# nv-tlabs/GEN3C

Hardware: NVIDIA H100
Metric: denoise-steps/sec, 7B DiT, 121-frame 720p latent (higher is better)
Workload: dtype bf16

## Files before the change

gen3c_b200/csrc/common.cuh:

```cuda
#pragma once
#include <cuda.h>
#include <cuda_bf16.h>
#include <cuda_runtime.h>
#include <stdint.h>
#include <stdio.h>

#include "../../include/gen3c_b200.h"
#include "wgmma_ops.cuh"

namespace g3c {

void set_error(const char* fmt, ...);
int cuda_fail(cudaError_t e, const char* what, const char* file, int line);
#define G3C_CUDA(x)                                                         \
  do {                                                                      \
    cudaError_t _e = (x);                                                   \
    if (_e != cudaSuccess) return ::g3c::cuda_fail(_e, #x, __FILE__, __LINE__); \
  } while (0)
#define G3C_REQUIRE(cond, ...)        \
  do {                                \
    if (!(cond)) {                    \
      ::g3c::set_error(__VA_ARGS__);  \
      return G3C_EINVAL;       \
    }                                 \
  } while (0)

int make_tmap_bf16_sw128(CUtensorMap* out, const void* base, int rank, const uint64_t* dims,
                         const uint64_t* strides_bytes, const uint32_t* box,
                         CUtensorMapDataType dtype = CU_TENSOR_MAP_DATA_TYPE_BFLOAT16);
int make_tmap_f32_sw128(CUtensorMap* out, const void* base, const uint64_t* dims,
                        const uint64_t* strides_bytes, const uint32_t* box);

int sm_count();

#ifdef __CUDACC__
__device__ __forceinline__ uint32_t smem_u32(const void* p) {
  return static_cast<uint32_t>(__cvta_generic_to_shared(p));
}
__device__ __forceinline__ uint32_t lane_id() { return threadIdx.x & 31; }
__device__ __forceinline__ uint32_t warp_id() { return __shfl_sync(0xffffffffu, threadIdx.x >> 5, 0); }

__device__ __forceinline__ bool elect_one() {
  uint32_t pred = 0;
  asm volatile(
      "{\n\t.reg .pred P;\n\t"
      "elect.sync _|P, 0xffffffff;\n\t"
      "selp.b32 %0, 1, 0, P;\n\t}\n"
      : "=r"(pred));
  return pred != 0;
}

__device__ __forceinline__ void mbar_init(uint64_t* bar, uint32_t count) {
  asm volatile("mbarrier.init.shared::cta.b64 [%0], %1;\n" ::"r"(smem_u32(bar)), "r"(count));
}
__device__ __forceinline__ void fence_barrier_init() {
  asm volatile("fence.mbarrier_init.release.cluster;\n" ::: "memory");
}
__device__ __forceinline__ void fence_proxy_async() {
  asm volatile("fence.proxy.async.shared::cta;\n" ::: "memory");
}
__device__ __forceinline__ void mbar_expect_tx(uint64_t* bar, uint32_t bytes) {
  asm volatile("mbarrier.arrive.expect_tx.shared::cta.b64 _, [%0], %1;\n" ::"r"(smem_u32(bar)),
               "r"(bytes)
               : "memory");
}
__device__ __forceinline__ void mbar_arrive(uint64_t* bar) {
  asm volatile("mbarrier.arrive.shared::cta.b64 _, [%0];\n" ::"r"(smem_u32(bar)) : "memory");
}
#ifndef G3C_MBAR_SUSPEND_NS
#define G3C_MBAR_SUSPEND_NS 0
#endif
__device__ __forceinline__ bool mbar_try_wait(uint64_t* bar, uint32_t parity) {
  uint32_t ok;
#if G3C_MBAR_SUSPEND_NS > 0
  asm volatile(
      "{\n\t.reg .pred P;\n\t"
      "mbarrier.try_wait.parity.shared::cta.b64 P, [%1], %2, %3;\n\t"
      "selp.b32 %0, 1, 0, P;\n\t}\n"
      : "=r"(ok)
      : "r"(smem_u32(bar)), "r"(parity), "r"((uint32_t)G3C_MBAR_SUSPEND_NS)
      : "memory");
#else
  asm volatile(
      "{\n\t.reg .pred P;\n\t"
      "mbarrier.try_wait.parity.shared::cta.b64 P, [%1], %2;\n\t"
      "selp.b32 %0, 1, 0, P;\n\t}\n"
      : "=r"(ok)
      : "r"(smem_u32(bar)), "r"(parity)
      : "memory");
#endif
  return ok != 0;
}
__device__ __forceinline__ bool mbar_test(uint64_t* bar, uint32_t parity) {
  uint32_t ok;
  asm volatile(
      "{\n\t.reg .pred P;\n\t"
      "mbarrier.test_wait.parity.shared::cta.b64 P, [%1], %2;\n\t"
      "selp.b32 %0, 1, 0, P;\n\t}\n"
      : "=r"(ok)
      : "r"(smem_u32(bar)), "r"(parity)
      : "memory");
  return ok != 0;
}
#ifndef G3C_MBAR_TIMEOUT_NS
#define G3C_MBAR_TIMEOUT_NS 4000000000ull
#endif
__device__ __forceinline__ uint64_t global_timer_ns() {
  uint64_t t;
  asm volatile("mov.u64 %0, %%globaltimer;\n" : "=l"(t));
  return t;
}
#ifdef G3C_MBAR_DEBUG
#define G3C_MBAR_TIMEOUT_ACTION(bar, parity)                                                                 \
  do {                                                                                                       \
    printf("g3c: mbarrier timeout block(%d,%d) thread %d bar@%u parity %u\n", blockIdx.x, blockIdx.y,        \
           threadIdx.x, bar, parity);                                                                        \
    __trap();                                                                                                \
  } while (0)
#else
#define G3C_MBAR_TIMEOUT_ACTION(bar, parity) asm volatile("trap;\n")
#endif
__device__ __forceinline__ void mbar_wait(uint64_t* bar, uint32_t parity) {
  if (mbar_try_wait(bar, parity)) return;
  uint32_t spins = 0;
  uint64_t t0 = 0;
  while (!mbar_try_wait(bar, parity)) {
    if ((++spins & 0xFFFu) == 0) {
      uint64_t now = global_timer_ns();
      if (t0 == 0) t0 = now;
      else if (now - t0 > G3C_MBAR_TIMEOUT_NS) G3C_MBAR_TIMEOUT_ACTION(smem_u32(bar), parity);
    }
  }
}

__device__ __forceinline__ void mbar_wait_ns(uint64_t* bar, uint32_t parity, unsigned long long timeout_ns) {
  if (mbar_try_wait(bar, parity)) return;
  uint32_t spins = 0;
  uint64_t t0 = 0;
  while (!mbar_try_wait(bar, parity)) {
    if ((++spins & 0xFFFu) == 0) {
      uint64_t now = global_timer_ns();
      if (t0 == 0) t0 = now;
      else if (now - t0 > timeout_ns) G3C_MBAR_TIMEOUT_ACTION(smem_u32(bar), parity);
    }
  }
}

__device__ __forceinline__ void mbar_wait_ns_or_exit(uint64_t* bar, uint32_t parity, unsigned long long timeout_ns) {
  if (mbar_try_wait(bar, parity)) return;
  uint32_t spins = 0;
  uint64_t t0 = 0;
  while (!mbar_try_wait(bar, parity)) {
    if ((++spins & 0xFFFu) == 0) {
      uint64_t now = global_timer_ns();
      if (t0 == 0) t0 = now;
      else if (now - t0 > timeout_ns) asm volatile("exit;\n");
    }
  }
}

__device__ __forceinline__ void tma_prefetch_desc(const CUtensorMap* m) {
  asm volatile("prefetch.tensormap [%0];\n" ::"l"(reinterpret_cast<uint64_t>(m)) : "memory");
}
__device__ __forceinline__ void tma_load_2d(void* smem_dst, const CUtensorMap* m, uint64_t* bar,
                                            int c0, int c1) {
  asm volatile(
      "cp.async.bulk.tensor.2d.shared::cluster.global.mbarrier::complete_tx::bytes"
      " [%0], [%1, {%3, %4}], [%2];\n" ::"r"(smem_u32(smem_dst)),
      "l"(reinterpret_cast<uint64_t>(m)), "r"(smem_u32(bar)), "r"(c0), "r"(c1)
      : "memory");
}
__device__ __forceinline__ void tma_load_3d(void* smem_dst, const CUtensorMap* m, uint64_t* bar,
                                            int c0, int c1, int c2) {
  asm volatile(
      "cp.async.bulk.tensor.3d.shared::cluster.global.mbarrier::complete_tx::bytes"
      " [%0], [%1, {%3, %4, %5}], [%2];\n" ::"r"(smem_u32(smem_dst)),
      "l"(reinterpret_cast<uint64_t>(m)), "r"(smem_u32(bar)), "r"(c0), "r"(c1), "r"(c2)
      : "memory");
}

__device__ __forceinline__ void tma_store_2d(const CUtensorMap* m, const void* smem_src, int c0, int c1) {
  asm volatile("cp.async.bulk.tensor.2d.global.shared::cta.bulk_group [%0, {%2, %3}], [%1];\n" ::"l"(
                   reinterpret_cast<uint64_t>(m)),
               "r"(smem_u32(smem_src)), "r"(c0), "r"(c1)
               : "memory");
}
__device__ __forceinline__ void tma_reduce_add_2d(const CUtensorMap* m, const void* smem_src, int c0, int c1) {
  asm volatile("cp.reduce.async.bulk.tensor.2d.global.shared::cta.add.bulk_group [%0, {%2, %3}], [%1];\n" ::"l"(
                   reinterpret_cast<uint64_t>(m)),
               "r"(smem_u32(smem_src)), "r"(c0), "r"(c1)
               : "memory");
}
__device__ __forceinline__ void tma_store_commit() { asm volatile("cp.async.bulk.commit_group;\n" ::: "memory"); }
template <int N>
__device__ __forceinline__ void tma_store_wait_read() {
  asm volatile("cp.async.bulk.wait_group.read %0;\n" ::"n"(N) : "memory");
}
template <int N>
__device__ __forceinline__ void tma_store_wait_all() {
  asm volatile("cp.async.bulk.wait_group %0;\n" ::"n"(N) : "memory");
}

__device__ __forceinline__ void wgmma_fence() { asm volatile("wgmma.fence.sync.aligned;\n" ::: "memory"); }
__device__ __forceinline__ void wgmma_commit() { asm volatile("wgmma.commit_group.sync.aligned;\n" ::: "memory"); }
template <int N>
__device__ __forceinline__ void wgmma_wait() {
  asm volatile("wgmma.wait_group.sync.aligned %0;\n" ::"n"(N) : "memory");
}
template <int N>
__device__ __forceinline__ void fence_regs(float (&r)[N]) {
#pragma unroll
  for (int i = 0; i < N; ++i) asm volatile("" : "+f"(r[i])::"memory");
}
template <int N>
__device__ __forceinline__ void fence_regs(uint32_t (&r)[N]) {
#pragma unroll
  for (int i = 0; i < N; ++i) asm volatile("" : "+r"(r[i])::"memory");
}

__device__ __forceinline__ uint64_t make_sdesc_sw128(uint32_t smem_addr) {
  uint64_t d = 0;
  d |= static_cast<uint64_t>((smem_addr & 0x3FFFFu) >> 4);
  d |= static_cast<uint64_t>(1) << 16;
  d |= static_cast<uint64_t>(1024u >> 4) << 32;
  d |= static_cast<uint64_t>(1) << 62;
  return d;
}
__device__ __forceinline__ uint64_t make_sdesc_sw128_mn(uint32_t smem_addr, uint32_t mn_block_bytes) {
  uint64_t d = 0;
  d |= static_cast<uint64_t>((smem_addr & 0x3FFFFu) >> 4);
  d |= static_cast<uint64_t>((mn_block_bytes >> 4) & 0x3FFFu) << 16;
  d |= static_cast<uint64_t>(1024u >> 4) << 32;
  d |= static_cast<uint64_t>(1) << 62;
  return d;
}
__device__ __forceinline__ uint64_t sdesc_advance(uint64_t d, uint32_t bytes) {
  return d + static_cast<uint64_t>(bytes >> 4);
}

template <int N>
__device__ __forceinline__ void setmaxnreg_dec() {
  asm volatile("setmaxnreg.dec.sync.aligned.u32 %0;\n" ::"n"(N));
}
template <int N>
__device__ __forceinline__ void setmaxnreg_inc() {
  asm volatile("setmaxnreg.inc.sync.aligned.u32 %0;\n" ::"n"(N));
}

__device__ __forceinline__ uint32_t pack_bf16x2(float lo, float hi) {
  __nv_bfloat162 v = __floats2bfloat162_rn(lo, hi);
  return *reinterpret_cast<uint32_t*>(&v);
}
__device__ __forceinline__ float warp_max(float v) {
#pragma unroll
  for (int o = 16; o > 0; o >>= 1) v = fmaxf(v, __shfl_xor_sync(0xffffffffu, v, o));
  return v;
}
__device__ __forceinline__ float warp_sum(float v) {
#pragma unroll
  for (int o = 16; o > 0; o >>= 1) v += __shfl_xor_sync(0xffffffffu, v, o);
  return v;
}
#endif

}
```

gen3c_b200/csrc/gemm_wgmma.cu:

```cuda
#include <cstdlib>
#include <cstring>

#include "kernels.h"

namespace g3c {

constexpr int BM = 128;
constexpr int BK = 64;
constexpr int WG_K = 16;
template <bool kFp8>
constexpr int kBlockK = kFp8 ? 2 * BK : BK;
constexpr int GEMM_THREADS = 384;

struct GemmParams {
  int M, N, K;
  int ldd;
  void* D;
  const float* gate;
  int num_m_blk, num_n_blk, num_k_blk;
  int super_n;
  const float* nr_gamma;
  const float* nr_cs;
  float nr_eps;
  const float* scale_a;
  const float* scale_b;
};

constexpr int EPI_NORM_ROPE_BF16 = 4;

template <int BN>
struct GemmSmem {
  static constexpr int kABytes = BM * BK * 2;
  static constexpr int kBBytes = BN * BK * 2;
  static constexpr int kStageBytes = kABytes + kBBytes;
  static constexpr int kStages = (192 * 1024) / kStageBytes;
  static constexpr int kBarBytes = 256;
  static constexpr int kTotal = kStages * kStageBytes + kBarBytes + 1024;
};

__device__ __forceinline__ float gelu_erf(float x) {
  return 0.5f * x * (1.0f + erff(x * 0.70710678118654752440f));
}

__device__ __forceinline__ void tile_coords(const GemmParams& p, int tile, int& m_blk, int& n_blk) {
  int per_super = p.num_m_blk * p.super_n;
  int sc = tile / per_super;
  int rem = tile - sc * per_super;
  int n0 = sc * p.super_n;
  int width = p.num_n_blk - n0 < p.super_n ? p.num_n_blk - n0 : p.super_n;
  m_blk = rem / width;
  n_blk = n0 + rem - m_blk * width;
}

template <int BN>
__device__ __forceinline__ void epilogue_norm_rope(const float (&acc)[BN / 2], const GemmParams& p, int row_a, int col_q,
                                                   int n_base) {
#pragma unroll
  for (int hd = 0; hd < BN / 128; ++hd) {
    if (n_base + hd * 128 >= p.N) break;
    float ss[2] = {0.f, 0.f};
#pragma unroll
    for (int i = 16 * hd; i < 16 * hd + 16; ++i) {
      ss[0] = fmaf(acc[4 * i], acc[4 * i], fmaf(acc[4 * i + 1], acc[4 * i + 1], ss[0]));
      ss[1] = fmaf(acc[4 * i + 2], acc[4 * i + 2], fmaf(acc[4 * i + 3], acc[4 * i + 3], ss[1]));
    }
#pragma unroll
    for (int h = 0; h < 2; ++h) {
      ss[h] += __shfl_xor_sync(0xffffffffu, ss[h], 1);
      ss[h] += __shfl_xor_sync(0xffffffffu, ss[h], 2);
    }
#pragma unroll
    for (int h = 0; h < 2; ++h) {
      const int row = row_a + 8 * h;
      if (row >= p.M) continue;
      const float rstd = rsqrtf(ss[h] * (1.0f / 128.0f) + p.nr_eps);
      const float* cs = p.nr_cs ? p.nr_cs + (size_t)row * 128 : nullptr;
      __nv_bfloat16* dptr = reinterpret_cast<__nv_bfloat16*>(p.D) + (size_t)row * p.ldd + n_base + hd * 128;
#pragma unroll
      for (int i = 0; i < 8; ++i) {
        const int c = 8 * i + col_q;
        const float2 ga = *reinterpret_cast<const float2*>(p.nr_gamma + c);
        const float2 gb = *reinterpret_cast<const float2*>(p.nr_gamma + 64 + c);
        const int ia = 4 * (16 * hd + i) + 2 * h, ib = 4 * (16 * hd + i + 8) + 2 * h;
        float a[2] = {acc[ia] * (rstd * ga.x), acc[ia + 1] * (rstd * ga.y)};
        float b[2] = {acc[ib] * (rstd * gb.x), acc[ib + 1] * (rstd * gb.y)};
        if (cs) {
          const float2 co = *reinterpret_cast<const float2*>(cs + c);
          const float2 si = *reinterpret_cast<const float2*>(cs + 64 + c);
          const float cv[2] = {co.x, co.y}, sv[2] = {si.x, si.y};
#pragma unroll
          for (int e = 0; e < 2; ++e) {
            const float n = a[e] * cv[e] - b[e] * sv[e], m = b[e] * cv[e] + a[e] * sv[e];
            a[e] = n;
            b[e] = m;
          }
        }
        *reinterpret_cast<uint32_t*>(dptr + c) = pack_bf16x2(a[0], a[1]);
        *reinterpret_cast<uint32_t*>(dptr + 64 + c) = pack_bf16x2(b[0], b[1]);
      }
    }
  }
}

template <int BN>
__device__ __forceinline__ void dequantise(float (&acc)[BN / 2], const GemmParams& p, int row_a, int col_q, int n_base) {
  float sa[2];
#pragma unroll
  for (int h = 0; h < 2; ++h) sa[h] = row_a + 8 * h < p.M ? p.scale_a[row_a + 8 * h] : 0.f;
#pragma unroll
  for (int i = 0; i < BN / 8; ++i) {
    const int col = n_base + 8 * i + col_q;
    float2 sb = make_float2(0.f, 0.f);
    if (col + 1 < p.N) sb = *reinterpret_cast<const float2*>(p.scale_b + col);
    else if (col < p.N) sb.x = p.scale_b[col];
#pragma unroll
    for (int h = 0; h < 2; ++h) {
      acc[4 * i + 2 * h] = acc[4 * i + 2 * h] * sa[h] * sb.x;
      acc[4 * i + 2 * h + 1] = acc[4 * i + 2 * h + 1] * sa[h] * sb.y;
    }
  }
}

template <int BN, int EPI>
__device__ __forceinline__ void epilogue(const float (&acc)[BN / 2], const GemmParams& p, int row_a, int col_q,
                                         int n_base) {
  if constexpr (EPI == EPI_NORM_ROPE_BF16) {
    epilogue_norm_rope<BN>(acc, p, row_a, col_q, n_base);
  } else {
#pragma unroll
    for (int h = 0; h < 2; ++h) {
      const int row = row_a + 8 * h;
      if (row >= p.M) continue;
#pragma unroll
      for (int i = 0; i < BN / 8; ++i) {
        const int col = n_base + 8 * i + col_q;
        if (col >= p.N) continue;
        const bool pair = col + 1 < p.N;
        float v0 = acc[4 * i + 2 * h], v1 = acc[4 * i + 2 * h + 1];
        if constexpr (EPI == G3C_EPI_BF16 || EPI == G3C_EPI_GELU_BF16) {
          if constexpr (EPI == G3C_EPI_GELU_BF16) {
            v0 = gelu_erf(v0);
            v1 = gelu_erf(v1);
          }
          __nv_bfloat16* dptr = reinterpret_cast<__nv_bfloat16*>(p.D) + (size_t)row * p.ldd + col;
          if (pair) *reinterpret_cast<uint32_t*>(dptr) = pack_bf16x2(v0, v1);
          else dptr[0] = __float2bfloat16_rn(v0);
        } else {
          float* dptr = reinterpret_cast<float*>(p.D) + (size_t)row * p.ldd + col;
          if constexpr (EPI == G3C_EPI_GATED_RESIDUAL_F32) {
            if (pair) {
              const float2 g = *reinterpret_cast<const float2*>(p.gate + col);
              float2 x = *reinterpret_cast<float2*>(dptr);
              x.x = fmaf(g.x, v0, x.x);
              x.y = fmaf(g.y, v1, x.y);
              *reinterpret_cast<float2*>(dptr) = x;
            } else {
              dptr[0] = fmaf(p.gate[col], v0, dptr[0]);
            }
          } else {
            if (pair) *reinterpret_cast<float2*>(dptr) = make_float2(v0, v1);
            else dptr[0] = v0;
          }
        }
      }
    }
  }
}

template <int BN, int EPI, bool kFp8>
__global__ void __launch_bounds__(GEMM_THREADS, 1)
    k_gemm(const __grid_constant__ CUtensorMap tmA, const __grid_constant__ CUtensorMap tmB, const GemmParams p) {
  using S = GemmSmem<BN>;
  constexpr int kStages = S::kStages;
  extern __shared__ uint8_t smem_raw[];
  uint8_t* smem = reinterpret_cast<uint8_t*>((reinterpret_cast<uintptr_t>(smem_raw) + 1023) &
                                             ~static_cast<uintptr_t>(1023));
  uint8_t* smem_a = smem;
  uint8_t* smem_b = smem + kStages * S::kABytes;
  uint64_t* bars = reinterpret_cast<uint64_t*>(smem + kStages * S::kStageBytes);
  uint64_t* full = bars;
  uint64_t* empty = bars + kStages;

  const uint32_t wg = threadIdx.x / 128;
  const uint32_t tid = threadIdx.x % 128;

  if (threadIdx.x == 0) {
    tma_prefetch_desc(&tmA);
    tma_prefetch_desc(&tmB);
    for (int i = 0; i < kStages; ++i) {
      mbar_init(&full[i], 1);
      mbar_init(&empty[i], 2);
    }
    fence_barrier_init();
  }
  __syncthreads();

  const int num_tiles = p.num_m_blk * p.num_n_blk;

  if (wg == 0) {
    setmaxnreg_dec<40>();
    if (tid == 0) {
      uint32_t stage = 0, phase = 0;
      for (int tile = blockIdx.x; tile < num_tiles; tile += gridDim.x) {
        int m_blk, n_blk;
        tile_coords(p, tile, m_blk, n_blk);
        for (int kb = 0; kb < p.num_k_blk; ++kb) {
          mbar_wait(&empty[stage], phase ^ 1);
          mbar_expect_tx(&full[stage], S::kStageBytes);
          tma_load_2d(smem_a + stage * S::kABytes, &tmA, &full[stage], kb * kBlockK<kFp8>, m_blk * BM);
          tma_load_2d(smem_b + stage * S::kBBytes, &tmB, &full[stage], kb * kBlockK<kFp8>, n_blk * BN);
          if (++stage == kStages) {
            stage = 0;
            phase ^= 1;
          }
        }
      }
    }
  } else {
    setmaxnreg_inc<232>();
    const uint32_t c = wg - 1;
    const uint32_t warp = tid / 32, lane = tid % 32;
    uint32_t stage = 0, phase = 0;
    float acc[BN / 2];
    for (int tile = blockIdx.x; tile < num_tiles; tile += gridDim.x) {
      int m_blk, n_blk;
      tile_coords(p, tile, m_blk, n_blk);
      if constexpr (kFp8) {
        static_assert(BN <= 128, "fp8 tiles hold two accumulator sets");
        float part[BN / 2];
#pragma unroll
        for (int i = 0; i < BN / 2; ++i) acc[i] = 0.f;
        for (int kb = 0; kb < p.num_k_blk; ++kb) {
          mbar_wait(&full[stage], phase);
          const uint64_t da = make_sdesc_sw128(smem_u32(smem_a + stage * S::kABytes + c * 64 * 128));
          const uint64_t db = make_sdesc_sw128(smem_u32(smem_b + stage * S::kBBytes));
          wgmma_fence();
#pragma unroll
          for (int k = 0; k < BK / WG_K; ++k) {
            const uint64_t a = sdesc_advance(da, k * WG_K * 2), b = sdesc_advance(db, k * WG_K * 2);
            if constexpr (BN == 128) wgmma_ss_n128_e4m3(part, a, b, k != 0 ? 1u : 0u);
            else wgmma_ss_n64_e4m3(part, a, b, k != 0 ? 1u : 0u);
          }
          wgmma_commit();
          wgmma_wait<0>();
          fence_regs(part);
          if (tid == 0) mbar_arrive(&empty[stage]);
#pragma unroll
          for (int i = 0; i < BN / 2; ++i) acc[i] += part[i];
          if (++stage == kStages) {
            stage = 0;
            phase ^= 1;
          }
        }
      } else {
        uint32_t prev_stage = 0;
        for (int kb = 0; kb < p.num_k_blk; ++kb) {
          mbar_wait(&full[stage], phase);
          const uint64_t da = make_sdesc_sw128(smem_u32(smem_a + stage * S::kABytes + c * 64 * 128));
          const uint64_t db = make_sdesc_sw128(smem_u32(smem_b + stage * S::kBBytes));
          wgmma_fence();
#pragma unroll
          for (int k = 0; k < BK / WG_K; ++k) {
            const uint64_t a = sdesc_advance(da, k * WG_K * 2), b = sdesc_advance(db, k * WG_K * 2);
            const uint32_t accumulate = (kb | k) != 0 ? 1u : 0u;
            if constexpr (BN == 256) wgmma_ss_n256(acc, a, b, accumulate);
            else if constexpr (BN == 128) wgmma_ss_n128(acc, a, b, accumulate);
            else wgmma_ss_n64(acc, a, b, accumulate);
          }
          wgmma_commit();
          wgmma_wait<1>();
          fence_regs(acc);
          if (kb > 0 && tid == 0) mbar_arrive(&empty[prev_stage]);
          prev_stage = stage;
          if (++stage == kStages) {
            stage = 0;
            phase ^= 1;
          }
        }
        wgmma_wait<0>();
        fence_regs(acc);
        if (tid == 0) mbar_arrive(&empty[prev_stage]);
      }
      const int row_a = m_blk * BM + (int)(c * 64 + warp * 16 + lane / 4), col_q = (int)(2 * (lane % 4));
      if constexpr (kFp8) dequantise<BN>(acc, p, row_a, col_q, n_blk * BN);
      epilogue<BN, EPI>(acc, p, row_a, col_q, n_blk * BN);
    }
  }
}

template <int BN, int EPI, bool kFp8>
static int launch_gemm(const CUtensorMap& tmA, const CUtensorMap& tmB, const GemmParams& p, cudaStream_t st) {
  using S = GemmSmem<BN>;
  static bool configured = false;
  if (!configured) {
    G3C_CUDA(cudaFuncSetAttribute(k_gemm<BN, EPI, kFp8>, cudaFuncAttributeMaxDynamicSharedMemorySize, S::kTotal));
    configured = true;
  }
  int tiles = p.num_m_blk * p.num_n_blk;
  int grid = tiles < sm_count() ? tiles : sm_count();
  k_gemm<BN, EPI, kFp8><<<grid, GEMM_THREADS, S::kTotal, st>>>(tmA, tmB, p);
  G3C_CUDA(cudaGetLastError());
  return G3C_OK;
}

template <int BN, bool kFp8>
static int dispatch_epi(int epi, const CUtensorMap& tmA, const CUtensorMap& tmB, const GemmParams& p, cudaStream_t st) {
  switch (epi) {
    case G3C_EPI_BF16: return launch_gemm<BN, G3C_EPI_BF16, kFp8>(tmA, tmB, p, st);
    case G3C_EPI_GELU_BF16: return launch_gemm<BN, G3C_EPI_GELU_BF16, kFp8>(tmA, tmB, p, st);
    case G3C_EPI_GATED_RESIDUAL_F32: return launch_gemm<BN, G3C_EPI_GATED_RESIDUAL_F32, kFp8>(tmA, tmB, p, st);
    case G3C_EPI_F32: return launch_gemm<BN, G3C_EPI_F32, kFp8>(tmA, tmB, p, st);
    case EPI_NORM_ROPE_BF16:
      if constexpr (BN >= 128) return launch_gemm<BN, EPI_NORM_ROPE_BF16, kFp8>(tmA, tmB, p, st);
      break;
  }
  set_error("gemm: unknown epilogue %d", epi);
  return G3C_EINVAL;
}

static int gemm_any(const void* A, const void* B, const float* scale_a, const float* scale_b, void* D, int M, int N,
                    int K, int lda, int ldb, int ldd, int epilogue, const float* gate, int block_n, cudaStream_t st,
                    const NormRope* norm_rope) {
  const bool fp8 = scale_a != nullptr;
  G3C_REQUIRE(A && B && D, "gemm: null operand");
  G3C_REQUIRE(epilogue >= G3C_EPI_BF16 && epilogue <= G3C_EPI_F32, "gemm: unknown epilogue %d", epilogue);
  if (norm_rope) {
    G3C_REQUIRE(epilogue == G3C_EPI_BF16 && N % 128 == 0 && norm_rope->gamma,
                "gemm: the RMSNorm/RoPE epilogue needs the bf16 epilogue, N %% 128 == 0 and a gain vector");
    G3C_REQUIRE((reinterpret_cast<uintptr_t>(norm_rope->gamma) & 15) == 0 &&
                    (reinterpret_cast<uintptr_t>(norm_rope->cs) & 15) == 0,
                "gemm: RMSNorm gain / RoPE table must be 16-byte aligned");
    epilogue = EPI_NORM_ROPE_BF16;
  }
  G3C_REQUIRE(M > 0 && N > 0 && K > 0, "gemm: bad shape %dx%dx%d", M, N, K);
  if (fp8)
    G3C_REQUIRE(K % 16 == 0 && lda % 16 == 0 && ldb % 16 == 0, "gemm_fp8: K/lda/ldb must be multiples of 16");
  else
    G3C_REQUIRE(K % 8 == 0 && lda % 8 == 0 && ldb % 8 == 0, "gemm: K/lda/ldb must be multiples of 8");
  G3C_REQUIRE(lda >= K && ldb >= K && ldd >= N, "gemm: leading dimension smaller than extent");
  if (epilogue == G3C_EPI_BF16 || epilogue == G3C_EPI_GELU_BF16 || epilogue == EPI_NORM_ROPE_BF16)
    G3C_REQUIRE(ldd % 8 == 0 && (reinterpret_cast<uintptr_t>(D) & 15) == 0,
                "gemm: bf16 output needs ldd %% 8 == 0 and 16-byte aligned base");
  else
    G3C_REQUIRE(ldd % 4 == 0 && (reinterpret_cast<uintptr_t>(D) & 15) == 0,
                "gemm: f32 output needs ldd %% 4 == 0 and 16-byte aligned base");
  G3C_REQUIRE(epilogue != G3C_EPI_GATED_RESIDUAL_F32 ||
                  (gate && (reinterpret_cast<uintptr_t>(gate) & 15) == 0),
              "gemm: gated-residual epilogue needs a 16-byte aligned gate vector");
  int bn = block_n;
  G3C_REQUIRE(bn == 0 || bn == 64 || bn == 128 || bn == 256 || bn == 512, "gemm: block_n %d unsupported", bn);
  if (bn == 512) {
    G3C_REQUIRE(N % 256 == 0, "gemm: block_n 512 needs N %% 256 == 0 (N=%d)", N);
    bn = 256;
  }
  if (bn == 0) bn = (N >= 256 && N % 256 == 0) ? 256 : (N > 64 ? 128 : 64);
  if (fp8 && bn == 256) bn = 128;
  G3C_REQUIRE(epilogue != EPI_NORM_ROPE_BF16 || bn >= 128, "gemm: the RMSNorm/RoPE epilogue needs tiles of whole heads");

  CUtensorMap tmA, tmB;
  const int esize = fp8 ? 1 : 2, bk = fp8 ? kBlockK<true> : kBlockK<false>;
  const CUtensorMapDataType dt = fp8 ? CU_TENSOR_MAP_DATA_TYPE_UINT8 : CU_TENSOR_MAP_DATA_TYPE_BFLOAT16;
  uint64_t dimsA[2] = {(uint64_t)K, (uint64_t)M}, strA[1] = {(uint64_t)lda * esize};
  uint32_t boxA[2] = {(uint32_t)bk, BM};
  int rc = make_tmap_bf16_sw128(&tmA, A, 2, dimsA, strA, boxA, dt);
  if (rc) return rc;
  uint64_t dimsB[2] = {(uint64_t)K, (uint64_t)N}, strB[1] = {(uint64_t)ldb * esize};
  uint32_t boxB[2] = {(uint32_t)bk, (uint32_t)bn};
  rc = make_tmap_bf16_sw128(&tmB, B, 2, dimsB, strB, boxB, dt);
  if (rc) return rc;

  GemmParams p;
  p.M = M;
  p.N = N;
  p.K = K;
  p.ldd = ldd;
  p.D = D;
  p.gate = gate;
  p.nr_gamma = norm_rope ? norm_rope->gamma : nullptr;
  p.nr_cs = norm_rope ? norm_rope->cs : nullptr;
  p.nr_eps = norm_rope ? norm_rope->eps : 0.0f;
  p.scale_a = scale_a;
  p.scale_b = scale_b;
  p.num_m_blk = (M + BM - 1) / BM;
  p.num_n_blk = (N + bn - 1) / bn;
  p.num_k_blk = (K + bk - 1) / bk;
  long long col_bytes = (long long)bn * K * esize;
  int sn = (int)((16ll << 20) / (col_bytes > 0 ? col_bytes : 1));
  if (sn < 1) sn = 1;
  if (sn > p.num_n_blk) sn = p.num_n_blk;
  p.super_n = sn;
  if (fp8) return bn == 64 ? dispatch_epi<64, true>(epilogue, tmA, tmB, p, st)
                           : dispatch_epi<128, true>(epilogue, tmA, tmB, p, st);
  switch (bn) {
    case 64: return dispatch_epi<64, false>(epilogue, tmA, tmB, p, st);
    case 128: return dispatch_epi<128, false>(epilogue, tmA, tmB, p, st);
    default: return dispatch_epi<256, false>(epilogue, tmA, tmB, p, st);
  }
}

int gemm_bf16(const void* A, const void* B, void* D, int M, int N, int K, int lda, int ldb, int ldd,
              int epilogue, const float* gate, int block_n, cudaStream_t st, const NormRope* norm_rope) {
  return gemm_any(A, B, nullptr, nullptr, D, M, N, K, lda, ldb, ldd, epilogue, gate, block_n, st, norm_rope);
}

int gemm_fp8(const void* A8, const float* scale_a, const void* B8, const float* scale_b, void* D, int M, int N, int K,
             int lda, int ldb, int ldd, int epilogue, const float* gate, int block_n, cudaStream_t st,
             const NormRope* norm_rope) {
  G3C_REQUIRE(scale_a && scale_b, "gemm_fp8: null scale vector");
  G3C_REQUIRE((reinterpret_cast<uintptr_t>(scale_a) & 15) == 0 && (reinterpret_cast<uintptr_t>(scale_b) & 15) == 0,
              "gemm_fp8: scale vectors must be 16-byte aligned");
  return gemm_any(A8, B8, scale_a, scale_b, D, M, N, K, lda, ldb, ldd, epilogue, gate, block_n, st, norm_rope);
}

}

extern "C" int g3c_gemm_bf16(const void* A, const void* B, void* D, int M, int N, int K, int lda,
                             int ldb, int ldd, int epilogue, const float* gate, int block_n,
                             void* stream) {
  return g3c::gemm_bf16(A, B, D, M, N, K, lda, ldb, ldd, epilogue, gate, block_n,
                        (cudaStream_t)stream);
}

extern "C" int g3c_gemm_fp8(const void* A8, const float* scale_A, const void* B8, const float* scale_B, void* D, int M,
                            int N, int K, int lda, int ldb, int ldd, int epilogue, const float* gate, int block_n,
                            void* stream) {
  return g3c::gemm_fp8(A8, scale_A, B8, scale_B, D, M, N, K, lda, ldb, ldd, epilogue, gate, block_n,
                       (cudaStream_t)stream);
}

extern "C" int g3c_gemm_norm_rope_fp8(const void* A8, const float* scale_A, const void* B8, const float* scale_B, void* D,
                                      int M, int N, int K, int lda, int ldb, int ldd, const float* gamma,
                                      const float* cos_sin, float eps, void* stream) {
  g3c::NormRope nr;
  nr.gamma = gamma;
  nr.cs = cos_sin;
  nr.eps = eps;
  return g3c::gemm_fp8(A8, scale_A, B8, scale_B, D, M, N, K, lda, ldb, ldd, G3C_EPI_BF16, nullptr, 0,
                       (cudaStream_t)stream, &nr);
}

extern "C" int g3c_gemm_norm_rope_bf16(const void* A, const void* B, void* D, int M, int N, int K, int lda, int ldb,
                                       int ldd, const float* gamma, const float* cos_sin, float eps, void* stream) {
  g3c::NormRope nr;
  nr.gamma = gamma;
  nr.cs = cos_sin;
  nr.eps = eps;
  return g3c::gemm_bf16(A, B, D, M, N, K, lda, ldb, ldd, G3C_EPI_BF16, nullptr, 0, (cudaStream_t)stream, &nr);
}
```

Baseline: 0.1368.

## Pair CTAs in clusters and multicast B tiles via TMA

GEMM CTAs now run in 2-CTA clusters that share an N tile across two adjacent M blocks. Each CTA loads half of the B tile and multicasts it to both CTAs, and the empty barriers count arrivals from both CTAs. The super-N grouping is now chosen by a small HBM-traffic model, and the gated-residual epilogue batches its gate and residual loads. This aims to cut L2/HBM traffic for B, at the cost of cross-CTA coupling that can stall one CTA on its partner and odd-M edge cases.

```diff
diff --git a/gen3c_b200/csrc/common.cuh b/gen3c_b200/csrc/common.cuh
--- a/gen3c_b200/csrc/common.cuh
+++ b/gen3c_b200/csrc/common.cuh
@@ -67,6 +67,23 @@
 __device__ __forceinline__ void mbar_arrive(uint64_t* bar) {
   asm volatile("mbarrier.arrive.shared::cta.b64 _, [%0];\n" ::"r"(smem_u32(bar)) : "memory");
 }
+__device__ __forceinline__ void mbar_arrive_cluster(uint64_t* bar, uint32_t rank) {
+  asm volatile(
+      "{\n\t.reg .b32 remote;\n\t"
+      "mapa.shared::cluster.u32 remote, %0, %1;\n\t"
+      "mbarrier.arrive.shared::cluster.b64 _, [remote];\n\t}\n" ::"r"(smem_u32(bar)),
+      "r"(rank)
+      : "memory");
+}
+
+__device__ __forceinline__ uint32_t cluster_ctarank() {
+  uint32_t r;
+  asm volatile("mov.u32 %0, %%cluster_ctarank;\n" : "=r"(r));
+  return r;
+}
+__device__ __forceinline__ void cluster_sync() {
+  asm volatile("barrier.cluster.arrive.release;\n\tbarrier.cluster.wait.acquire;\n" ::: "memory");
+}
 #ifndef G3C_MBAR_SUSPEND_NS
 #define G3C_MBAR_SUSPEND_NS 0
 #endif
@@ -170,6 +187,14 @@
       "l"(reinterpret_cast<uint64_t>(m)), "r"(smem_u32(bar)), "r"(c0), "r"(c1)
       : "memory");
 }
+__device__ __forceinline__ void tma_load_2d_multicast(void* smem_dst, const CUtensorMap* m, uint64_t* bar, int c0,
+                                                      int c1, uint16_t cta_mask) {
+  asm volatile(
+      "cp.async.bulk.tensor.2d.shared::cluster.global.mbarrier::complete_tx::bytes.multicast::cluster"
+      " [%0], [%1, {%4, %5}], [%2], %3;\n" ::"r"(smem_u32(smem_dst)),
+      "l"(reinterpret_cast<uint64_t>(m)), "r"(smem_u32(bar)), "h"(cta_mask), "r"(c0), "r"(c1)
+      : "memory");
+}
 __device__ __forceinline__ void tma_load_3d(void* smem_dst, const CUtensorMap* m, uint64_t* bar,
                                             int c0, int c1, int c2) {
   asm volatile(
diff --git a/gen3c_b200/csrc/gemm_wgmma.cu b/gen3c_b200/csrc/gemm_wgmma.cu
--- a/gen3c_b200/csrc/gemm_wgmma.cu
+++ b/gen3c_b200/csrc/gemm_wgmma.cu
@@ -18,6 +18,7 @@
   void* D;
   const float* gate;
   int num_m_blk, num_n_blk, num_k_blk;
+  int num_pairs;
   int super_n;
   const float* nr_gamma;
   const float* nr_cs;
@@ -42,14 +43,14 @@
   return 0.5f * x * (1.0f + erff(x * 0.70710678118654752440f));
 }
 
-__device__ __forceinline__ void tile_coords(const GemmParams& p, int tile, int& m_blk, int& n_blk) {
-  int per_super = p.num_m_blk * p.super_n;
+__device__ __forceinline__ void tile_coords(const GemmParams& p, int tile, int& pair, int& n_blk) {
+  int per_super = p.num_pairs * p.super_n;
   int sc = tile / per_super;
   int rem = tile - sc * per_super;
   int n0 = sc * p.super_n;
   int width = p.num_n_blk - n0 < p.super_n ? p.num_n_blk - n0 : p.super_n;
-  m_blk = rem / width;
-  n_blk = n0 + rem - m_blk * width;
+  pair = rem / width;
+  n_blk = n0 + rem - pair * width;
 }
 
 template <int BN>
@@ -121,11 +122,60 @@
   }
 }
 
+template <int BN>
+__device__ __forceinline__ void epilogue_gated(const float (&acc)[BN / 2], const GemmParams& p, int row_a, int col_q,
+                                               int n_base) {
+  constexpr int kChunk = 8;
+  static_assert((BN / 8) % kChunk == 0, "whole chunks of column pairs");
+  float* rows[2];
+  bool live[2];
+#pragma unroll
+  for (int h = 0; h < 2; ++h) {
+    live[h] = row_a + 8 * h < p.M;
+    rows[h] = reinterpret_cast<float*>(p.D) + (size_t)(live[h] ? row_a + 8 * h : 0) * p.ldd;
+  }
+#pragma unroll
+  for (int i0 = 0; i0 < BN / 8; i0 += kChunk) {
+    float2 g[kChunk], x[2][kChunk];
+#pragma unroll
+    for (int j = 0; j < kChunk; ++j) {
+      const int col = n_base + 8 * (i0 + j) + col_q;
+      g[j] = make_float2(0.f, 0.f);
+      if (col + 1 < p.N) g[j] = *reinterpret_cast<const float2*>(p.gate + col);
+      else if (col < p.N) g[j].x = p.gate[col];
+#pragma unroll
+      for (int h = 0; h < 2; ++h) {
+        x[h][j] = make_float2(0.f, 0.f);
+        if (!live[h]) continue;
+        if (col + 1 < p.N) x[h][j] = *reinterpret_cast<const float2*>(rows[h] + col);
+        else if (col < p.N) x[h][j].x = rows[h][col];
+      }
+    }
+#pragma unroll
+    for (int j = 0; j < kChunk; ++j) {
+      const int i = i0 + j, col = n_base + 8 * i + col_q;
+#pragma unroll
+      for (int h = 0; h < 2; ++h) {
+        if (!live[h] || col >= p.N) continue;
+        const float y0 = fmaf(g[j].x, acc[4 * i + 2 * h], x[h][j].x);
+        if (col + 1 < p.N) {
+          const float y1 = fmaf(g[j].y, acc[4 * i + 2 * h + 1], x[h][j].y);
+          *reinterpret_cast<float2*>(rows[h] + col) = make_float2(y0, y1);
+        } else {
+          rows[h][col] = y0;
+        }
+      }
+    }
+  }
+}
+
 template <int BN, int EPI>
 __device__ __forceinline__ void epilogue(const float (&acc)[BN / 2], const GemmParams& p, int row_a, int col_q,
                                          int n_base) {
   if constexpr (EPI == EPI_NORM_ROPE_BF16) {
     epilogue_norm_rope<BN>(acc, p, row_a, col_q, n_base);
+  } else if constexpr (EPI == G3C_EPI_GATED_RESIDUAL_F32) {
+    epilogue_gated<BN>(acc, p, row_a, col_q, n_base);
   } else {
 #pragma unroll
     for (int h = 0; h < 2; ++h) {
@@ -147,20 +197,8 @@
           else dptr[0] = __float2bfloat16_rn(v0);
         } else {
           float* dptr = reinterpret_cast<float*>(p.D) + (size_t)row * p.ldd + col;
-          if constexpr (EPI == G3C_EPI_GATED_RESIDUAL_F32) {
-            if (pair) {
-              const float2 g = *reinterpret_cast<const float2*>(p.gate + col);
-              float2 x = *reinterpret_cast<float2*>(dptr);
-              x.x = fmaf(g.x, v0, x.x);
-              x.y = fmaf(g.y, v1, x.y);
-              *reinterpret_cast<float2*>(dptr) = x;
-            } else {
-              dptr[0] = fmaf(p.gate[col], v0, dptr[0]);
-            }
-          } else {
-            if (pair) *reinterpret_cast<float2*>(dptr) = make_float2(v0, v1);
-            else dptr[0] = v0;
-          }
+          if (pair) *reinterpret_cast<float2*>(dptr) = make_float2(v0, v1);
+          else dptr[0] = v0;
         }
       }
     }
@@ -183,32 +221,36 @@
 
   const uint32_t wg = threadIdx.x / 128;
   const uint32_t tid = threadIdx.x % 128;
+  const uint32_t rank = cluster_ctarank(), partner = rank ^ 1u;
+  const int cluster = (int)(blockIdx.x / 2), clusters = (int)(gridDim.x / 2);
 
   if (threadIdx.x == 0) {
     tma_prefetch_desc(&tmA);
     tma_prefetch_desc(&tmB);
     for (int i = 0; i < kStages; ++i) {
       mbar_init(&full[i], 1);
-      mbar_init(&empty[i], 2);
+      mbar_init(&empty[i], 4);
     }
     fence_barrier_init();
   }
-  __syncthreads();
-
-  const int num_tiles = p.num_m_blk * p.num_n_blk;
+  cluster_sync();
+
+  const int num_tiles = p.num_pairs * p.num_n_blk;
 
   if (wg == 0) {
     setmaxnreg_dec<40>();
     if (tid == 0) {
       uint32_t stage = 0, phase = 0;
-      for (int tile = blockIdx.x; tile < num_tiles; tile += gridDim.x) {
-        int m_blk, n_blk;
-        tile_coords(p, tile, m_blk, n_blk);
+      for (int tile = cluster; tile < num_tiles; tile += clusters) {
+        int pair, n_blk;
+        tile_coords(p, tile, pair, n_blk);
+        const int m_blk = 2 * pair + (int)rank;
         for (int kb = 0; kb < p.num_k_blk; ++kb) {
           mbar_wait(&empty[stage], phase ^ 1);
           mbar_expect_tx(&full[stage], S::kStageBytes);
           tma_load_2d(smem_a + stage * S::kABytes, &tmA, &full[stage], kb * kBlockK<kFp8>, m_blk * BM);
-          tma_load_2d(smem_b + stage * S::kBBytes, &tmB, &full[stage], kb * kBlockK<kFp8>, n_blk * BN);
+          tma_load_2d_multicast(smem_b + stage * S::kBBytes + rank * (S::kBBytes / 2), &tmB, &full[stage],
+                                kb * kBlockK<kFp8>, n_blk * BN + (int)rank * (BN / 2), 0x3);
           if (++stage == kStages) {
             stage = 0;
             phase ^= 1;
@@ -222,9 +264,10 @@
     const uint32_t warp = tid / 32, lane = tid % 32;
     uint32_t stage = 0, phase = 0;
     float acc[BN / 2];
-    for (int tile = blockIdx.x; tile < num_tiles; tile += gridDim.x) {
-      int m_blk, n_blk;
-      tile_coords(p, tile, m_blk, n_blk);
+    for (int tile = cluster; tile < num_tiles; tile += clusters) {
+      int pair, n_blk;
+      tile_coords(p, tile, pair, n_blk);
+      const int m_blk = 2 * pair + (int)rank;
       if constexpr (kFp8) {
         static_assert(BN <= 128, "fp8 tiles hold two accumulator sets");
         float part[BN / 2];
@@ -244,7 +287,10 @@
           wgmma_commit();
           wgmma_wait<0>();
           fence_regs(part);
-          if (tid == 0) mbar_arrive(&empty[stage]);
+          if (tid == 0) {
+            mbar_arrive(&empty[stage]);
+            mbar_arrive_cluster(&empty[stage], partner);
+          }
 #pragma unroll
           for (int i = 0; i < BN / 2; ++i) acc[i] += part[i];
           if (++stage == kStages) {
@@ -270,7 +316,10 @@
           wgmma_commit();
           wgmma_wait<1>();
           fence_regs(acc);
-          if (kb > 0 && tid == 0) mbar_arrive(&empty[prev_stage]);
+          if (kb > 0 && tid == 0) {
+            mbar_arrive(&empty[prev_stage]);
+            mbar_arrive_cluster(&empty[prev_stage], partner);
+          }
           prev_stage = stage;
           if (++stage == kStages) {
             stage = 0;
@@ -279,27 +328,78 @@
         }
         wgmma_wait<0>();
         fence_regs(acc);
-        if (tid == 0) mbar_arrive(&empty[prev_stage]);
+        if (tid == 0) {
+          mbar_arrive(&empty[prev_stage]);
+          mbar_arrive_cluster(&empty[prev_stage], partner);
+        }
       }
       const int row_a = m_blk * BM + (int)(c * 64 + warp * 16 + lane / 4), col_q = (int)(2 * (lane % 4));
       if constexpr (kFp8) dequantise<BN>(acc, p, row_a, col_q, n_blk * BN);
       epilogue<BN, EPI>(acc, p, row_a, col_q, n_blk * BN);
     }
   }
+  cluster_sync();
+}
+
+constexpr long long kL2Budget = 16ll << 20;
+
+static double hbm_bytes_model(const GemmParams& p, int w, int clusters, double a_all, long long b_blk) {
+  double total = 0;
+  for (int n0 = 0; n0 < p.num_n_blk; n0 += w) {
+    const int width = p.num_n_blk - n0 < w ? p.num_n_blk - n0 : w;
+    double b = (double)width * b_blk;
+    if (width * b_blk > kL2Budget) {
+      const long long waves = ((long long)p.num_pairs * width + clusters - 1) / clusters;
+      b = (double)waves * (width < clusters ? width : clusters) * b_blk;
+    }
+    total += a_all + b;
+  }
+  return total;
+}
+
+static int choose_super_n(const GemmParams& p, int clusters, int bn, int esize) {
+  const double a_all = (double)p.M * p.K * esize;
+  const long long b_blk = (long long)bn * p.K * esize;
+  int best = 1;
+  double best_bytes = hbm_bytes_model(p, 1, clusters, a_all, b_blk);
+  for (int w = 2; w <= p.num_n_blk; ++w) {
+    const double b = hbm_bytes_model(p, w, clusters, a_all, b_blk);
+    if (b < best_bytes) {
+      best = w;
+      best_bytes = b;
+    }
+  }
+  return best;
 }
 
 template <int BN, int EPI, bool kFp8>
-static int launch_gemm(const CUtensorMap& tmA, const CUtensorMap& tmB, const GemmParams& p, cudaStream_t st) {
+static int launch_gemm(const CUtensorMap& tmA, const CUtensorMap& tmB, GemmParams p, cudaStream_t st) {
   using S = GemmSmem<BN>;
-  static bool configured = false;
-  if (!configured) {
+  static int max_clusters = 0;
+  cudaLaunchAttribute attr[1];
+  attr[0].id = cudaLaunchAttributeClusterDimension;
+  attr[0].val.clusterDim.x = 2;
+  attr[0].val.clusterDim.y = 1;
+  attr[0].val.clusterDim.z = 1;
+  cudaLaunchConfig_t cfg = {};
+  cfg.blockDim = dim3(GEMM_THREADS);
+  cfg.dynamicSmemBytes = S::kTotal;
+  cfg.stream = st;
+  cfg.attrs = attr;
+  cfg.numAttrs = 1;
+  if (max_clusters == 0) {
     G3C_CUDA(cudaFuncSetAttribute(k_gemm<BN, EPI, kFp8>, cudaFuncAttributeMaxDynamicSharedMemorySize, S::kTotal));
-    configured = true;
-  }
-  int tiles = p.num_m_blk * p.num_n_blk;
-  int grid = tiles < sm_count() ? tiles : sm_count();
-  k_gemm<BN, EPI, kFp8><<<grid, GEMM_THREADS, S::kTotal, st>>>(tmA, tmB, p);
-  G3C_CUDA(cudaGetLastError());
+    cfg.gridDim = dim3(2 * (sm_count() / 2));
+    int n = 0;
+    G3C_CUDA(cudaOccupancyMaxActiveClusters(&n, k_gemm<BN, EPI, kFp8>, &cfg));
+    G3C_REQUIRE(n > 0, "gemm: no cluster of two CTAs fits the device");
+    max_clusters = n;
+  }
+  const int tiles = p.num_pairs * p.num_n_blk;
+  const int clusters = tiles < max_clusters ? tiles : max_clusters;
+  p.super_n = choose_super_n(p, clusters, BN, kFp8 ? 1 : 2);
+  cfg.gridDim = dim3(2 * clusters);
+  G3C_CUDA(cudaLaunchKernelEx(&cfg, k_gemm<BN, EPI, kFp8>, tmA, tmB, p));
   return G3C_OK;
 }
 
@@ -365,7 +465,7 @@
   int rc = make_tmap_bf16_sw128(&tmA, A, 2, dimsA, strA, boxA, dt);
   if (rc) return rc;
   uint64_t dimsB[2] = {(uint64_t)K, (uint64_t)N}, strB[1] = {(uint64_t)ldb * esize};
-  uint32_t boxB[2] = {(uint32_t)bk, (uint32_t)bn};
+  uint32_t boxB[2] = {(uint32_t)bk, (uint32_t)bn / 2};
   rc = make_tmap_bf16_sw128(&tmB, B, 2, dimsB, strB, boxB, dt);
   if (rc) return rc;
 
@@ -384,11 +484,8 @@
   p.num_m_blk = (M + BM - 1) / BM;
   p.num_n_blk = (N + bn - 1) / bn;
   p.num_k_blk = (K + bk - 1) / bk;
-  long long col_bytes = (long long)bn * K * esize;
-  int sn = (int)((16ll << 20) / (col_bytes > 0 ? col_bytes : 1));
-  if (sn < 1) sn = 1;
-  if (sn > p.num_n_blk) sn = p.num_n_blk;
-  p.super_n = sn;
+  p.num_pairs = (p.num_m_blk + 1) / 2;
+  p.super_n = 1;
   if (fp8) return bn == 64 ? dispatch_epi<64, true>(epilogue, tmA, tmB, p, st)
                            : dispatch_epi<128, true>(epilogue, tmA, tmB, p, st);
   switch (bn) {
```

New measurement: 0.1416 (median of 6 runs). 1.04x the previous value.
